# pierremtb/PINNs-TF2.0

Hardware: AMD Instinct MI355X
Metric: collocation-points/sec (higher is better)
Workload: dtype f64

## Files before the change

### pinns-tf2.0_amd/csrc/engine.hip

```cpp
#include <hip/hip_runtime.h>
#include <rccl/rccl.h>

#include <cmath>
#include <cstdarg>
#include <cstddef>
#include <cstdio>
#include <cstring>
#include <string>
#include <chrono>
#include <type_traits>
#include <vector>

#include "../../include/pinn_hip.h"
#include "devbuf.h"
#include "optim_host.h"
#include "kernels_fused20.h"
#include "kernels_fused20m.h"
#include "fused20d_api.h"
#include "fused20m_api.h"
#include "kernels_wide.h"
#include "kernels_generic.h"
#include "kernels_optim.h"
#include "kernels_disc.h"
#include "kernels_sampling.h"
// ... 87 lines not shown

struct pinn_ctx {
  int device = 0, dtype = PINN_F32, pde = PINN_PDE_BURGERS;
  KernelPath path = KP_GENERIC;
  hipStream_t stream = nullptr;
  bool own_stream = true;
  NetDesc nd{};
  int layers[MAX_DENSE + 1]{};
  int n_layers = 0;
  double lb[2]{}, ub[2]{}, nu = 0.0;
  double adr[6]{};
  int adr_mask = 0;

  PointSets sets;
  int64_t nf_total = 0, nu_total = 0, nb_total = 0;
  bool sets_dirty = true;
  SetDesc sd{};

  DevBuf<void> xs, ts, tgt;
  DevBuf<double> theta, gl, adam_m, adam_v;
  DevBuf<void> theta_r;
  DevBuf<float> img;
  DevBuf<int> row_index;
  int n_cu = 256, n_wg = 0;
  int f64_split = -1;
  DevBuf<void> S, O, ZA, ZB, part;
  int chunk = 0, n_rows = 0, R = 0;
  DevBuf<void> xe, te, Oe;
  DevBuf<double> f_out;
  std::vector<double> ev_X, ev_ref;
  int ev_n_pad = 0;
  DevBuf<double> pred, d_ref, err_partial, err_res;
  PinnedBuf<double> h_err;
  DevBuf<unsigned long long> d_nonfinite;
  unsigned long long n_evals = 0;

  struct {
    double lr = 1e-3, b1 = 0.9, b2 = 0.999, eps = 1e-7;
    int64_t t = 0;
    bool ready = false, want_terms = false;
    DevBuf<double> loss_hist;
    size_t hist_stride = 0;
  } adam;

  struct Pending {
    int kind = 0;
    int n = 0;
    int base = 0, issued_upto = 0;
    bool want_terms = false;
    hipEvent_t ev = nullptr;
    PinnedBuf<double> h_loss;
    PinnedBuf<int> h_iter;
    PinnedBuf<LbfgsState> h_state;
  };
  static constexpr int N_SNAP = 4;
  DevBuf<double> snap;
  unsigned snap_valid = 0;
  struct : Tickets { Pending pend[N_PENDING]; } tk;

  struct {
    int issued_at_read = 0;
    DevBuf<LbfgsState> state;
    int flip = 0;
    DevBuf<double> x, d, gold, S, Y, ro, al, q, log_loss;
    DevBuf<int> log_iter;
    int max_iter = 0, ncorr = 0, logged_read = 0;
    double lr = 1.0, tol_fun = 0, tol_x = 0, max_eval = 0;
    int iters_issued = 0;
    bool post_pending = false;
    bool ready = false;
    int mode = 1, mode_active = 0, M1 = 0;
    DevBuf<double> SY, YY, dots, cs, cy;
    DevBuf<LbcExtra> ex;
  } lbfgs;
  double t16_cost_full = T16_COST_FULL, t16_cost_strip = T16_COST_STRIP;
  long long t16_handover_ticks = 50000000ll;
  bool t16_prepass_pinned = false;
  bool t16_prepass = false;
  DevBuf<unsigned int> t16_bsync;
  unsigned int t16_bcount = 0;
  DevBuf<double> t16_gscr;

  enum ColFrom { COL_HANDED, COL_LHS, COL_RAD };
  struct ColOrigin { ColFrom from = COL_HANDED; int64_t n_design = 0, first = 0, count = 0; } col;
  struct { uint64_t seed = 0; } lhs;
  struct {
    bool filled = false;
    DevBuf<double> cx, ct;
    DevBuf<void> px, pt, O;
    DevBuf<double> f;
    DevBuf<unsigned long long> w, bsum;
    DevBuf<RadTotals> tot;
  } rad;

  struct {
    bool on = false;
    double lr = 0.0;
    LamStore arr;
  } sa;
  struct {
    bool on = false;
    double rate[3] = {0.0, 0.0, 0.0};
    LamStore arr;
  } pw;

  struct {
    std::vector<double> X, alpha, beta, g;
    int64_t n_total = 0;
    DevBuf<void> ab;
    int first = 0, n = 0;
    DevBuf<double> out;
  } robin;

  struct {
    std::vector<double> s;
    bool on = false, stale = false;
  } src;

  struct {
    std::vector<double> K;
    bool on = false, stale = false;
    DevBuf<void> dev;
// ... 782 lines not shown
  HIPCHK(hipMemsetAsync(c->part, 0, need_part, c->stream));
  c->dd = dd;
  c->n_rows = G;
  c->sets_dirty = false;
  return 0;
}

template <typename real, int NT>
static int disc_set_lds() {
  static unsigned long long done = 0;
  if (!first_call_on_device(done)) return 0;
  HIPCHK(hipFuncSetAttribute((const void*)k_disc_fwd<real, NT>, hipFuncAttributeMaxDynamicSharedMemorySize,
                             (int)disc_fwd_lds<NT>(sizeof(real))));
  HIPCHK(hipFuncSetAttribute((const void*)k_disc_bwd_out<real, NT>, hipFuncAttributeMaxDynamicSharedMemorySize,
                             (int)disc_out_lds<NT>(sizeof(real))));
  HIPCHK(hipFuncSetAttribute((const void*)k_disc_bwd_hidden<real, NT>, hipFuncAttributeMaxDynamicSharedMemorySize,
                             (int)disc_hid_lds<NT>(sizeof(real))));
  return 0;
}

template <typename real, int NT>
static int disc_eval(pinn_ctx* c, hipEvent_t* ev4, const AdamFuse* af) {
  const DiscDesc dd = c->dd;
  const InMap<real> m(c->lb, c->ub);
  const real c1 = real(1), c2 = (real)c->nu;
  if (int rc = disc_set_lds<real, NT>()) return rc;
  const dim3 grid(dd.n_groups, dd.n_chunks), block(256);
  const real* th = c->theta_r.as<real>();
  if (ev4) HIPCHK(hipEventRecord(ev4[0], c->stream));
  hipLaunchKernelGGL((k_disc_fwd<real, NT>), grid, block, disc_fwd_lds<NT>(sizeof(real)), c->stream, c->nd, dd, th,
                     c->xs.as<real>(), m.lbx, m.sx, c1, c2, c->d_Ast.as<real>(), c->d_A3.as<real>(), c->d_U3.as<real>(),
                     c->d_Nn.as<real>(), 1);
  hipLaunchKernelGGL((k_disc_irk<real>), grid, block, 0, c->stream, dd, c->nd.n_out, c->d_ginfo,
                     c->d_MT[0].as<real>(), c->d_MT[1].as<real>(), c->d_Nn.as<real>(),
                     c->d_U3.as<real>(), c->tgt.as<real>(), c->d_R.as<real>(), c->d_lossp.as<real>(), 0);
  if (ev4) HIPCHK(hipEventRecord(ev4[1], c->stream));
  hipLaunchKernelGGL((k_disc_bwd_out<real, NT>), grid, block, disc_out_lds<NT>(sizeof(real)), c->stream, c->nd, dd,
                     th, c->d_ginfo, c->d_M[0].as<real>(), c->d_M[1].as<real>(), c->d_R.as<real>(),
                     c->d_U3.as<real>(), c->d_A3.as<real>(), c1, c2, c->part.as<real>(), c->R, c->d_dAp.as<real>(),
                     c->d_lamp.as<real>());
  hipLaunchKernelGGL((k_disc_bwd_hidden<real, NT>), dim3(dd.n_groups), block, disc_hid_lds<NT>(sizeof(real)),
                     c->stream, c->nd, dd, th, c->d_ginfo, c->xs.as<real>(), m.lbx, m.sx, c->d_Ast.as<real>(),
                     c->d_dAp.as<real>(), c->d_lossp.as<real>(), c->d_lamp.as<real>(), c->part.as<real>(), c->R);
  if (ev4) HIPCHK(hipEventRecord(ev4[2], c->stream));
  HIPCHK(hipGetLastError());
  return launch_reduce<real>(c, dd.n_groups, af);
}

static int disc_eval_any(pinn_ctx* c, hipEvent_t* ev4, const AdamFuse* af) {
  if (c->dtype == PINN_F64) return disc_eval<double, 4>(c, ev4, af);
  return c->dd.wp == 64 ? disc_eval<float, 4>(c, ev4, af) : disc_eval<float, 8>(c, ev4, af);
}

static int eval_loss_grad(pinn_ctx* c, const AdamFuse* af = nullptr) {
  int rc = src_fresh(c, "evaluation");
  if (rc) return rc;
  rc = is_disc(c) ? disc_ensure(c) : ensure_sets(c);
  if (rc) return rc;
  c->n_evals += 1;
  hipEvent_t* ev4 = nullptr;
  if (c->timing && c->ev_used < c->ev_cap_evals && (c->ev_seen++ % c->ev_every) == 0)
    ev4 = &c->ev[(size_t)4 * c->ev_used];
  if (is_disc(c)) rc = disc_eval_any(c, ev4, af);
  else
    rc = by_kind(c, pde_kind(c, AT_TRAINING), [&](auto r, auto kind) {
      return launch_sweeps<decltype(r), decltype(kind)::value>(c, ev4, af);
    });
  if (rc) return rc;
  if (c->comm && !c->xg.on)
    NCCLCHK(ncclAllReduce(c->gl, c->gl, (size_t)c->R, ncclDouble, ncclSum, c->comm, c->stream));
  if (ev4) { HIPCHK(hipEventRecord(ev4[3], c->stream)); c->ev_used++; }
  return 0;
}

template <typename real, int NT>
static int disc_predict_impl(pinn_ctx* c, int mode, int set, const double* x, int64_t n, double* out) {
  const int NO = c->nd.n_out;
  const int G = (int)((n + 15) / 16);
  DiscDesc dd{};
  disc_layout(c, dd, G, mode == 1 && c->dset[set].has_M ? c->dset[set].q : 0);
  std::vector<double> hx(dd.n_pad, c->lb[0]);
  for (int64_t i = 0; i < n; ++i) hx[i] = x[i];
  std::vector<int> gi(G, disc_ginfo(set, 16));
  DevBuf<void> xe, U3, Nn, Rb;
  DevBuf<int> ge;
  const size_t rs = sizeof(real);
  HIPCHK(xe.reserve_bytes(dd.n_pad * rs));
  HIPCHK(ge.reserve(G));
  if (disc_alloc_scratch(c, dd, nullptr, nullptr, U3, Nn, Rb)) return PINN_EHIP;
  if (upload_real(c, xe, hx.data(), dd.n_pad)) return PINN_EHIP;
  if (hipMemcpy(ge, gi.data(), G * sizeof(int), hipMemcpyHostToDevice) != hipSuccess) return PINN_EHIP;
  const InMap<real> m(c->lb, c->ub);
  const size_t lds_f = disc_fwd_lds<NT>(rs);
  if (int rc = disc_set_lds<real, NT>()) return rc;
  const dim3 grid(dd.n_groups, dd.n_chunks), block(256);
  hipLaunchKernelGGL((k_disc_fwd<real, NT>), grid, block, lds_f, c->stream, c->nd, dd, c->theta_r.as<real>(),
                     xe.as<real>(), m.lbx, m.sx, real(1), (real)c->nu, (real*)nullptr, (real*)nullptr, U3.as<real>(),
                     Nn.as<real>(), 0);
  if (mode == 1)
    hipLaunchKernelGGL((k_disc_irk<real>), grid, block, 0, c->stream, dd, NO, ge.get(), c->d_MT[0].as<real>(),
                       c->d_MT[1].as<real>(), Nn.as<real>(), U3.as<real>(), (const real*)nullptr, Rb.as<real>(),
                       (real*)nullptr, 1);
  std::vector<real> ho((size_t)dd.n_pad * dd.ldo);
  if (hipMemcpyAsync(ho.data(), mode == 1 ? Rb.get() : U3.get(), ho.size() * rs, hipMemcpyDeviceToHost, c->stream) != hipSuccess ||
      hipStreamSynchronize(c->stream) != hipSuccess)
    return fail(PINN_EHIP, "discrete-time predict failed: %s", hipGetErrorString(hipGetLastError()));
  for (int64_t i = 0; i < n; ++i)
    for (int j = 0; j < NO; ++j) out[(size_t)i * NO + j] = (double)ho[(size_t)i * dd.ldo + j];
  return 0;
}

// ... 900 lines not shown
  if (int rc = xg_check(c)) return rc;
  if (losses) {
    if (p.want_terms) memcpy(losses, p.h_loss, (size_t)3 * p.n * 8);
    else for (int s = 0; s < p.n; ++s) losses[s] = p.h_loss[3 * s] + p.h_loss[3 * s + 1] + p.h_loss[3 * s + 2];
  }
  return 0;
}

int pinn_adam_run(pinn_ctx* c, int n_steps, double* losses) {
  REQUIRE(c && n_steps >= 0, "bad arguments");
  if (n_steps == 0) return 0;
  if (!losses) return adam_issue(c, n_steps, false, nullptr);
  REQUIRE(c->tk.outstanding() == 0, "pinn_adam_run: %d chunk(s) are in flight; collect them first", c->tk.outstanding());
  int ticket = 0;
  if (int rc = adam_issue(c, n_steps, true, &ticket)) return rc;
  return pinn_adam_collect(c, ticket, losses);
}

int pinn_adam_enqueue(pinn_ctx* c, int n_steps, int* ticket) {
  REQUIRE(c && ticket && n_steps >= 1, "bad arguments");
  return adam_issue(c, n_steps, true, ticket);
}

int pinn_adam_enqueue_terms(pinn_ctx* c, int n_steps, int* ticket) {
  REQUIRE(c && ticket && n_steps >= 1, "bad arguments");
  c->adam.want_terms = true;
  const int rc = adam_issue(c, n_steps, true, ticket);
  c->adam.want_terms = false;
  return rc;
}

int pinn_adam_run_terms(pinn_ctx* c, int n_steps, double* terms3) {
  REQUIRE(c && terms3, "null");
  c->adam.want_terms = true;
  const int rc = pinn_adam_run(c, n_steps, terms3);
  c->adam.want_terms = false;
  return rc;
}

static int lbfgs_begin_setup(pinn_ctx* c, int max_iter, double lr, int n_corr, double tol_fun, double tol_x,
                             double max_eval, bool* eval) {
  *eval = false;
  REQUIRE(c && max_iter >= 0 && n_corr >= 1 && lr > 0, "bad L-BFGS arguments");
  if (int rc0 = src_fresh(c, "pinn_lbfgs_begin")) return rc0;
  HIPCHK(hipSetDevice(c->device));
  const size_t n = c->nd.n_theta;
  auto& lb = c->lbfgs;
  lb.max_iter = max_iter; lb.lr = lr; lb.ncorr = n_corr; lb.tol_fun = tol_fun; lb.tol_x = tol_x;
  lb.max_eval = max_eval > 0 ? max_eval : 1.25 * max_iter;
  if (c->tk.outstanding() > 0) {
    HIPCHK(hipStreamSynchronize(c->stream));
    c->tk.drop_all();
  }
  lb.iters_issued = 0; lb.logged_read = 0; lb.issued_at_read = 0; lb.post_pending = false; lb.ready = false;
  if (max_iter == 0) { lb.ready = true; return 0; }
  const int M1 = lb.M1 = n_corr + 1;
  lb.mode_active = (lb.mode == 1 && M1 <= LBC_MAXSLOTS) ? 1 : 0;
  if (lb.mode_active && lbc_coef_apply_lds_bytes(M1) > 64 * 1024) {
    const int lds = (int)lbc_coef_apply_lds_bytes(M1);
    HIPCHK(hipFuncSetAttribute((const void*)k_lbc_coef_apply<float>, hipFuncAttributeMaxDynamicSharedMemorySize, lds));
    HIPCHK(hipFuncSetAttribute((const void*)k_lbc_coef_apply<double>, hipFuncAttributeMaxDynamicSharedMemorySize, lds));
  }
  const size_t m1 = M1, ring = m1 * ring_ld((int)n), gram = 2 * m1 * m1, dots = 2 * (5 * m1 + LBC_NSCAL);
  const struct { DevBuf<double>* buf; size_t count; bool zero; } bufs[] = {
      {&lb.x, n, false},    {&lb.d, n, false},    {&lb.gold, n, false},  {&lb.q, n, false},     {&lb.al, m1, false},
      {&lb.S, ring, true},  {&lb.Y, ring, true},  {&lb.cs, m1, true},    {&lb.cy, m1, true},    {&lb.SY, gram, true},
      {&lb.YY, gram, true}, {&lb.ro, 2 * m1, true}, {&lb.dots, dots, true}};
  static_assert(sizeof(LbcExtra) % 8 == 0, "LbcExtra is cleared as doubles");
  ZeroList zl{};
  auto add = [&](void* p, size_t doubles) { zl.p[zl.count] = (double*)p; zl.n[zl.count] = doubles; zl.count++; };
  for (const auto& b : bufs) {
    HIPCHK(b.buf->reserve(b.count));
    if (b.zero) add(b.buf->get(), b.count);
  }
  HIPCHK(lb.state.reserve(2));
  HIPCHK(lb.ex.reserve(1));
  add(lb.ex, sizeof(LbcExtra) / 8);
  static_assert(sizeof(LbfgsState) % 8 == 0 && offsetof(LbfgsState, Hdiag) % 8 == 0, "LbfgsState is initialised as doubles");
  zl.state = (double*)lb.state.get(); zl.state_doubles = (int)(sizeof(LbfgsState) / 8);
  zl.hdiag_index = (int)(offsetof(LbfgsState, Hdiag) / 8);
  hipLaunchKernelGGL(k_zero_list, dim3(256), dim3(256), 0, c->stream, zl);
  HIPCHK(hipGetLastError());
  lb.flip = 0;
  HIPCHK(lb.log_loss.reserve((size_t)max_iter + 1));
  HIPCHK(lb.log_iter.reserve((size_t)max_iter + 1));
  HIPCHK(hipMemcpyAsync(lb.x, c->theta, n * 8, hipMemcpyDeviceToDevice, c->stream));
  *eval = true;
  return 0;
}

static void lbfgs_post(pinn_ctx* c, int initial) {
  const auto& lb = c->lbfgs;
  const int n = c->nd.n_theta;
  hipLaunchKernelGGL(k_lbfgs_post, dim3(1), dim3(LB_THREADS), 0, c->stream, n, n, lb.max_iter, lb.max_eval, lb.tol_fun,
                     lb.tol_x, lb.state + lb.flip, c->gl, lb.d, lb.log_iter, lb.log_loss, initial);
}

static int lbfgs_begin_post(pinn_ctx* c) {
  lbfgs_post(c, 1);
  HIPCHK(hipGetLastError());
  if (c->xg.on) {
    HIPCHK(hipStreamSynchronize(c->stream));
    if (int rc2 = xg_check(c)) return rc2;
  }
  c->lbfgs.ready = true;
  return 0;
}

int pinn_lbfgs_begin(pinn_ctx* c, int max_iter, double lr, int n_corr, double tol_fun,
                     double tol_x, double max_eval) {
  bool eval = false;
  if (int rc = lbfgs_begin_setup(c, max_iter, lr, n_corr, tol_fun, tol_x, max_eval, &eval)) return rc;
  if (!eval) return 0;
  if (int rc = eval_loss_grad(c)) return rc;
  return lbfgs_begin_post(c);
}

struct LbfgsMember { pinn_ctx* c; pinn_ctx::Pending* p; int window, ticket; };

static int lbfgs_open(LbfgsMember& m, int n_iters) {
  pinn_ctx* c = m.c;
  REQUIRE(c && n_iters >= 0, "bad arguments");
  if (int rc0 = src_fresh(c, "pinn_lbfgs_run / pinn_lbfgs_enqueue")) return rc0;
  const auto& lb = c->lbfgs;
  REQUIRE(lb.ready, "pinn_lbfgs_begin has not been called");
  HIPCHK(hipSetDevice(c->device));
  pinn_ctx::Pending* p = nullptr;
  const int log_room = (int)(lb.log_iter.capacity_bytes() / sizeof(int));
  const int window = lbfgs_window(lb.iters_issued, lb.issued_at_read, n_iters, log_room, lb.logged_read, lb.max_iter);
  if (int rc = pend_reserve(c, 2, (size_t)window + 1, (size_t)window + 1, true, &p)) return rc;
  if (lb.max_iter == 0) { p->n = -1; return ticket_issue(c, p, &m.ticket); }
  m.p = p; m.window = window;
  return 0;
}

static bool lbfgs_iter(pinn_ctx* c) {
  auto& lb = c->lbfgs;
  const int n = c->nd.n_theta;
  lb.iters_issued += 1;
  if (lb.mode_active) {
    const int M1 = lb.M1;
    const size_t lsh = lbc_coef_apply_lds_bytes(M1), mm = (size_t)M1 * M1;
    LbfgsState *st_in = lb.state + lb.flip, *st_out = lb.state + (lb.flip ^ 1);
    const int n_part = n <= 2 * 2 * LBD_THREADS ? 2 : 1;
    if (n_part == 2)
      hipLaunchKernelGGL(k_lbc_dots<2>, dim3(M1, 2), dim3(LBD_THREADS), 0, c->stream, n, M1, st_in, c->gl, lb.gold, lb.d,
                         lb.S, lb.Y, lb.dots);
    else
      hipLaunchKernelGGL(k_lbc_dots<1>, dim3(M1), dim3(LBD_THREADS), 0, c->stream, n, M1, st_in, c->gl, lb.gold, lb.d,
                         lb.S, lb.Y, lb.dots);
    const double* pd = lb.dots;
    const dim3 agrid((n + 63) / 64);
    by_real(c, [&](auto r) {
      using real = decltype(r);
      hipLaunchKernelGGL((k_lbc_coef_apply<real>), agrid, dim3(LBC_THREADS), lsh, c->stream, n, M1, lb.ncorr, lb.max_iter,
                         lb.lr, lb.tol_x, lb.tol_fun, lb.max_eval, lb.post_pending ? 1 : 0, n, st_in, st_out, c->gl, pd,
                         n_part, lb.SY + lb.flip * mm, lb.YY + lb.flip * mm, lb.ro + lb.flip * M1,
                         lb.SY + (lb.flip ^ 1) * mm, lb.YY + (lb.flip ^ 1) * mm, lb.ro + (lb.flip ^ 1) * M1, lb.log_iter,
                         lb.log_loss, lb.S, lb.Y, lb.d, lb.gold, lb.x, c->theta, c->theta_r.as<real>(), c->nd, c->img);
    });
    lb.post_pending = false;
    lb.flip ^= 1;
  } else
    by_real(c, [&](auto r) {
      using real = decltype(r);
      hipLaunchKernelGGL((k_lbfgs_step<real>), dim3(1), dim3(LB_THREADS), 0, c->stream, n, lb.max_iter, lb.ncorr,
                         lb.lr, lb.tol_x, lb.state + lb.flip, c->gl, lb.x, c->theta, c->theta_r.as<real>(),
                         lb.d, lb.gold, lb.S, lb.Y, lb.ro, lb.al, lb.q, c->nd, c->img);
    });
  return lb.iters_issued != lb.max_iter;
}

static int lbfgs_close(LbfgsMember& m) {
  pinn_ctx* c = m.c;
  auto& lb = c->lbfgs;
  pinn_ctx::Pending* p = m.p;
  if (lb.post_pending) { lbfgs_post(c, 0); lb.post_pending = false; }
  HIPCHK(hipGetLastError());
  p->n = m.window; p->base = lb.logged_read; p->issued_upto = lb.iters_issued;
  HIPCHK(hipMemcpyAsync(p->h_state, lb.state + lb.flip, sizeof(LbfgsState), hipMemcpyDeviceToHost, c->stream));
  if (m.window > 0) {
    HIPCHK(hipMemcpyAsync(p->h_iter, lb.log_iter + p->base, (size_t)m.window * 4, hipMemcpyDeviceToHost, c->stream));
    HIPCHK(hipMemcpyAsync(p->h_loss, lb.log_loss + p->base, (size_t)m.window * 8, hipMemcpyDeviceToHost, c->stream));
  }
  return ticket_issue(c, p, &m.ticket);
}

extern "C++" {
template <typename Eval>
static int lbfgs_chunk(LbfgsMember* m, char* act, int K, int n_iters, Eval&& eval) {
  for (int k = 0; k < K; ++k)
    if (int rc = lbfgs_open(m[k], n_iters)) return rc;
  for (int s = 0; s < n_iters; ++s) {
    bool any = false;
    for (int k = 0; k < K; ++k) {
      pinn_ctx* c = m[k].c;
      act[k] = m[k].p && c->lbfgs.iters_issued < c->lbfgs.max_iter && lbfgs_iter(c);
      any = any || act[k];
    }
    if (!any) break;
    if (int rc = eval(act)) return rc;
    for (int k = 0; k < K; ++k) {
      if (!act[k]) continue;
      if (m[k].c->lbfgs.mode_active) m[k].c->lbfgs.post_pending = true;
      else lbfgs_post(m[k].c, 0);
    }
  }
  for (int k = 0; k < K; ++k)
    if (m[k].p) { if (int rc = lbfgs_close(m[k])) return rc; }
  return 0;
}
}

static int lbfgs_issue(pinn_ctx* c, int n_iters, int* ticket) {
  const Range rg("pinn_lbfgs_run");
  LbfgsMember m{c, nullptr, 0, 0};
  char act = 0;
  if (int rc = lbfgs_chunk(&m, &act, 1, n_iters, [c](const char*) { return eval_loss_grad(c); })) return rc;
  *ticket = m.ticket;
  return 0;
}

int pinn_lbfgs_collect(pinn_ctx* c, int ticket, int cap, int* iters, double* losses, int* n_logged, int* done) {
  REQUIRE(cap >= 0, "bad arguments");
  pinn_ctx::Pending* pp = nullptr;
  if (int rc = ticket_oldest(c, ticket, 2, &pp)) return rc;
  const pinn_ctx::Pending& p = *pp;
  auto& lb = c->lbfgs;
  if (n_logged) *n_logged = 0;
  if (p.n < 0) { if (done) *done = 1; return 0; }
  if (int rc2 = xg_check(c)) return rc2;
  const LbfgsState hs = *p.h_state;
  const LbfgsHandout h = lbfgs_handout(hs.n_logged, lb.logged_read, p.base, p.n);
  REQUIRE(!(iters && losses) || h.fresh <= cap, "pinn_lbfgs_collect: %d log entries are due, the arrays hold %d", h.fresh, cap);
  if (h.fresh > 0 && iters && losses) {
    if (!h.inside)
      return fail(PINN_ESTATE, "pinn_lbfgs_collect: log entries from %d on lie outside the chunk's window of %d", h.off, p.n);
    memcpy(iters, p.h_iter + h.off, (size_t)h.fresh * 4);
    memcpy(losses, p.h_loss + h.off, (size_t)h.fresh * 8);
  }
  lb.logged_read = hs.n_logged;
  lb.issued_at_read = p.issued_upto;
  if (n_logged) *n_logged = (iters && losses) ? h.fresh : 0;
  if (done) *done = hs.done;
  return 0;
}

int pinn_lbfgs_run(pinn_ctx* c, int n_iters, int* iters, double* losses, int* n_logged, int* done) {
  REQUIRE(c && n_iters >= 0, "bad arguments");
  REQUIRE(c->tk.outstanding() == 0, "pinn_lbfgs_run: %d chunk(s) are in flight; collect them first", c->tk.outstanding());
  int ticket = 0;
  if (int rc = lbfgs_issue(c, n_iters, &ticket)) return rc;
  return pinn_lbfgs_collect(c, ticket, n_iters, iters, losses, n_logged, done);
}

int pinn_lbfgs_enqueue(pinn_ctx* c, int n_iters, int* ticket) {
  REQUIRE(c && ticket && n_iters >= 1, "bad arguments");
  return lbfgs_issue(c, n_iters, ticket);
}

int pinn_lbfgs_set_mode(pinn_ctx* c, int mode) {
  REQUIRE(c && (mode == 0 || mode == 1), "mode must be 0 (reference operation order) or 1 (compact)");
  c->lbfgs.mode = mode;
  return 0;
}

int pinn_lbfgs_get_x(pinn_ctx* c, double* x, int64_t n) {
  REQUIRE(c && x && n == c->nd.n_theta, "bad arguments");
  REQUIRE(c->lbfgs.x, "no L-BFGS run yet");
  HIPCHK(hipSetDevice(c->device));
  HIPCHK(hipMemcpyAsync(x, c->lbfgs.x, (size_t)n * 8, hipMemcpyDeviceToHost, c->stream));
  HIPCHK(hipStreamSynchronize(c->stream));
  return 0;
}

int pinn_predict(pinn_ctx* c, const double* X, int64_t n, double* out) {
  REQUIRE(c && X && out && n >= 0, "bad arguments");
  HIPCHK(hipSetDevice(c->device));
  if (n == 0) return 0;
  if (is_disc(c))
    return disc_predict_any(c, 0, 0, X, n, out);
  const Range rg("pinn_predict");
  int n_pad = 0;
  if (int rc = eval_points(c, X, n, &n_pad)) return rc;
  if (int rc = predict_values(c, n, n_pad)) return rc;
  HIPCHK(hipMemcpyAsync(out, c->pred, (size_t)n * c->nd.n_out * 8, hipMemcpyDeviceToHost, c->stream));
  HIPCHK(hipStreamSynchronize(c->stream));
  return 0;
}

int pinn_error_l2(pinn_ctx* c, const double* X, const double* ref, int64_t n, int kind, double* err) {
  REQUIRE(c && X && ref && err && n >= 1, "bad arguments");
// ... 930 lines not shown
}

int pinn_ens_adam_init(pinn_ens* e, double lr, double beta1, double beta2, double eps, const double* lr_k) {
  REQUIRE(e, "null");
  for (int k = 0; k < e->K; ++k)
    if (int rc = pinn_adam_init(e->mem[k], lr_k ? lr_k[k] : lr, beta1, beta2, eps)) return rc;
  return 0;
}

int pinn_ens_adam_run(pinn_ens* e, int n_steps, double* losses) {
  REQUIRE(e && n_steps >= 0, "bad arguments");
  for (pinn_ctx* c : e->mem) REQUIRE(c->adam.ready, "pinn_ens_adam_init has not been called");
  pinn_ctx* b = e->base;
  HIPCHK(hipSetDevice(b->device));
  if (n_steps == 0) return 0;
  const size_t K = e->K;
  HIPCHK(e->loss_hist.reserve((size_t)n_steps * K * 3));
  std::vector<char> all(K, 1);
  std::vector<double> alpha(K);
  for (int s = 0; s < n_steps; ++s) {
    for (size_t k = 0; k < K; ++k)
      alpha[k] = adam_step_factors(e->mem[k]).alpha(e->mem[k]->adam.lr);
    if (int rc = ens_eval(e, (const bool*)all.data(), alpha.data(), e->loss_hist + (size_t)s * K * 3)) return rc;
  }
  std::vector<double> h((size_t)n_steps * K * 3);
  HIPCHK(hipMemcpyAsync(h.data(), e->loss_hist, h.size() * 8, hipMemcpyDeviceToHost, b->stream));
  HIPCHK(hipStreamSynchronize(b->stream));
  if (losses)
    for (size_t i = 0; i < (size_t)n_steps * K; ++i) losses[i] = h[3 * i] + h[3 * i + 1] + h[3 * i + 2];
  return 0;
}

int pinn_ens_lbfgs_begin(pinn_ens* e, int n_corr, double tol_fun, double tol_x, double max_eval, double lr,
                         const double* lr_k, int max_iter, const int* max_iter_k) {
  REQUIRE(e, "null");
  REQUIRE(n_corr >= 1, "bad L-BFGS arguments");
  for (int k = 0; k < e->K; ++k) {
    REQUIRE((lr_k ? lr_k[k] : lr) > 0 && (max_iter_k ? max_iter_k[k] : max_iter) >= 0,
            "bad L-BFGS arguments for member %d", k);
  }
  HIPCHK(hipSetDevice(e->base->device));
  std::vector<char> ev((size_t)e->K, 0);
  bool any = false;
  for (int k = 0; k < e->K; ++k) {
    bool eval = false;
    if (int rc = lbfgs_begin_setup(e->mem[k], max_iter_k ? max_iter_k[k] : max_iter, lr_k ? lr_k[k] : lr, n_corr,
                                   tol_fun, tol_x, max_eval, &eval)) return rc;
    ev[k] = eval;
    any = any || eval;
  }
  if (!any) return 0;
  if (int rc = ens_eval(e, (const bool*)ev.data(), nullptr, nullptr)) return rc;
  for (int k = 0; k < e->K; ++k)
    if (ev[k]) { if (int rc = lbfgs_begin_post(e->mem[k])) return rc; }
  return 0;
}

int pinn_ens_lbfgs_run(pinn_ens* e, int n_iters, int* iters, double* losses, int* n_logged, int* done) {
  REQUIRE(e && n_iters >= 0, "bad arguments");
  for (pinn_ctx* c : e->mem) {
    REQUIRE(c->lbfgs.ready, "pinn_ens_lbfgs_begin has not been called");
    REQUIRE(c->tk.outstanding() == 0, "chunks in flight");
  }
  HIPCHK(hipSetDevice(e->base->device));
  const Range rg("pinn_ens_lbfgs_run");
  const int K = e->K;
  std::vector<LbfgsMember> m(K);
  for (int k = 0; k < K; ++k) m[k].c = e->mem[k];
  std::vector<char> act(K, 0);
  if (int rc = lbfgs_chunk(m.data(), act.data(), K, n_iters,
                           [e](const char* a) { return ens_eval(e, (const bool*)a, nullptr, nullptr); })) return rc;
  const int ld = n_iters + 1;
  for (int k = 0; k < K; ++k) {
    int nl = 0, dn = 0;
    if (int rc = pinn_lbfgs_collect(m[k].c, m[k].ticket, n_iters, iters ? iters + (size_t)k * ld : nullptr,
                               losses ? losses + (size_t)k * ld : nullptr, &nl, &dn)) return rc;
    if (n_logged) n_logged[k] = nl;
    if (done) done[k] = dn;
  }
  return 0;
}

int pinn_ens_predict(pinn_ens* e, const double* X, int64_t n, double* out) {
  REQUIRE(e && X && out && n >= 0, "bad arguments");
  for (int k = 0; k < e->K; ++k)
    if (int rc = pinn_predict(e->mem[k], X, n, out + (size_t)k * n)) return rc;
  return 0;
}

int pinn_ens_error_l2(pinn_ens* e, const double* X, const double* ref, int64_t n, double* err) {
  REQUIRE(e && X && ref && err && n > 0, "bad arguments");
  for (int k = 0; k < e->K; ++k)
    if (int rc = pinn_error_l2(e->mem[k], X, ref, n, 0, err + k)) return rc;
  return 0;
}

int pinn_ens_get_status(pinn_ens* e, int64_t* n_evals, int64_t* first_nonfinite_eval) {
  REQUIRE(e, "null");
  for (int k = 0; k < e->K; ++k) {
    int64_t a = 0, b = 0;
    if (int rc = pinn_get_status(e->mem[k], &a, &b)) return rc;
    if (n_evals) n_evals[k] = a;
    if (first_nonfinite_eval) first_nonfinite_eval[k] = b;
  }
  return 0;
}

// ... 2 lines not shown
```

### pinns-tf2.0_amd/csrc/kernels_optim.h

```cpp
#pragma once
#include "kernels_wide.h"

namespace pinn {

#ifndef PINN_REDUCE_ONE_ROUND
#define PINN_REDUCE_ONE_ROUND 1
#endif
constexpr int RED_COLS = 64;
constexpr int RED_SLICES = 16;
constexpr int RED_THREADS = RED_COLS * RED_SLICES;

template <typename real>
__device__ __forceinline__ double reduce_column(const real* __restrict__ part, int n_rows, int R,
                                                int c, int q, double (*sh)[RED_COLS]) {
  const int cl = threadIdx.x & 63;
  double a0 = 0, a1 = 0, a2 = 0, a3 = 0, a4 = 0, a5 = 0, a6 = 0, a7 = 0;
  if (c < R) {
#if PINN_REDUCE_ONE_ROUND
    const unsigned lane_off = (unsigned)c * (unsigned)sizeof(real);
    for (int r0 = __builtin_amdgcn_readfirstlane(q); r0 < n_rows; r0 += 16 * RED_SLICES) {
      real v[16];
#pragma unroll
      for (int i = 0; i < 16; ++i)
        v[i] = (r0 + i * RED_SLICES < n_rows)
// ... 384 lines not shown
    const double xi = x[i] + t * d[i];
    x[i] = xi;
    if (will_eval) { theta[i] = xi; theta_r[i] = (real)xi; pack_store_any(nd, img, i, (float)xi); }
  }
  if (tid == 0) {
    st->n_iter = n_iter; st->hist_len = hist_len; st->hist_head = head; st->Hdiag = Hdiag;
    st->t = t; st->f_old = st->f;
    if (!will_eval) st->done = 1;
  }
}

__global__ __launch_bounds__(LB_THREADS) void k_lbfgs_post(
    int n, int n_theta, int max_iter, double max_eval, double tol_fun, double tol_x,
    LbfgsState* __restrict__ st, const double* __restrict__ gl, const double* __restrict__ d,
    int* __restrict__ log_iters, double* __restrict__ log_losses, int initial) {
  __shared__ double sh[LB_THREADS / 64];
  if (st->done) return;
  const int tid = threadIdx.x;
  const double f = gl[n_theta] + gl[n_theta + 1] + gl[n_theta + 2];
  double ga_p = 0, sa_p = 0;
  const double t = st->t;
  for (int i = tid; i < n; i += LB_THREADS) {
    ga_p += fabs(gl[i]);
    if (!initial) sa_p += fabs(d[i] * t);
  }
  const double gabs = block_sum(ga_p, sh);
  const double sabs = block_sum(sa_p, sh);
  if (tid != 0) return;
  if (initial) {
    st->f = f; st->func_eval = 1;
    if (gabs <= tol_fun) st->done = 7;
    return;
  }
  const double f_old = st->f_old;
  st->f = f;
  st->func_eval += 1;
  const int n_iter = st->n_iter;
  if (n_iter == max_iter) { st->done = 1; return; }
  if ((double)st->func_eval >= max_eval) { st->done = 3; return; }
  if (gabs <= tol_fun) { st->done = 4; return; }
  if (sabs <= tol_x) { st->done = 5; return; }
  if (fabs(f - f_old) < tol_x) { st->done = 6; return; }
  const int k = st->n_logged;
  log_iters[k] = n_iter;
  log_losses[k] = f;
  st->n_logged = k + 1;
  if (n_iter == max_iter - 1) st->final_loss = f;
}

struct LbcExtra {
  int apply, will_eval, pad0, pad1;
  double cg, gtd;
};

struct ZeroList {
  double* p[10];
  unsigned long long n[10];
  int count;
  double* state;
  int state_doubles, hdiag_index;
};
__global__ __launch_bounds__(256) void k_zero_list(ZeroList zl) {
  if (zl.state && blockIdx.x == 0 && threadIdx.x == 0)
    for (int i = 0; i < zl.state_doubles; ++i) zl.state[i] = i == zl.hdiag_index ? 1.0 : 0.0;
  for (int a = 0; a < zl.count; ++a) {
    double* __restrict__ p = zl.p[a];
    const unsigned long long n = zl.n[a];
    for (unsigned long long i = (unsigned long long)blockIdx.x * 256 + threadIdx.x; i < n;
         i += (unsigned long long)gridDim.x * 256)
      p[i] = 0.0;
  }
}

constexpr int LBC_THREADS = 1024;
constexpr int LBC_ROWS = 4;
constexpr int LBD_THREADS = 1024;
constexpr int LBC_NSCAL = 5;

template <int NV>
__device__ __forceinline__ void block_sums(double (&v)[NV], double (*sh)[8]) {
  const int w = threadIdx.x >> 6;
#pragma unroll
  for (int i = 0; i < NV; ++i) {
    const double t = wave_sum(v[i]);
    if ((threadIdx.x & 63) == 0) sh[w][i] = t;
  }
  __syncthreads();
#pragma unroll
  for (int i = 0; i < NV; ++i) {
    double t = 0;
#pragma unroll
    for (int k = 0; k < LBD_THREADS / 64; ++k) t += sh[k][i];
    v[i] = t;
  }
}

template <int HALVES>
__global__ __launch_bounds__(LBD_THREADS) void k_lbc_dots(
    int n, int M1, const LbfgsState* __restrict__ st, const double* __restrict__ g,
    const double* __restrict__ g_old, const double* __restrict__ d, double* __restrict__ Sh,
    double* __restrict__ Yh, double* __restrict__ dots_all) {
  __shared__ double sh[LBD_THREADS / 64][8];
  double* __restrict__ dots = dots_all + (HALVES == 2 ? blockIdx.y * (5 * M1 + LBC_NSCAL) : 0);
  const int u0 = HALVES == 2 ? (int)blockIdx.y : 0;
  constexpr int NS = HALVES == 2 ? 1 : 2;
  typedef double d2 __attribute__((ext_vector_type(2)));
  const int a = blockIdx.x, tid = threadIdx.x;
  const int done0 = st->done, head = st->hist_head, len = st->hist_len, n_it = st->n_iter;
  const double t = st->t;
  d2 gv[NS], gov[NS], dv[NS], sav[NS], yav[NS];
#pragma unroll
  for (int u = 0; u < NS; ++u) {
    const int i = 2 * tid + (u0 + u) * 2 * LBD_THREADS;
    const d2 z = {0.0, 0.0};
    gv[u] = gov[u] = dv[u] = sav[u] = yav[u] = z;
    if (i + 1 < n) {
      gv[u] = *reinterpret_cast<const d2*>(g + i); gov[u] = *reinterpret_cast<const d2*>(g_old + i);
// ... 87 lines not shown
  extern __shared__ double lsh[];
  const int tid = threadIdx.x, lane = tid & 63, wave = uni(tid >> 6);
  const bool writer = blockIdx.x == 0;
  const int LD = M1 | 1;
  double* const sU = lsh;
  double* const sL = sU + M1 * LD;
  double* const sY = sL + M1 * LD;
  double* const sT = sY + M1 * LD;
  double* const sC = sT + 6 * 64;
  double* const sP = sC + 192;
  double* const sZ = sP + 16 * 64;
  CSTAMP(0);
  const bool in_row = lane < M1;
  const LbfgsState s0 = *st_in;
  int head = uni(s0.hist_head), len = uni(s0.hist_len);
  double Hdiag = s0.Hdiag, f_cur = s0.f;
  const int ndp = 5 * M1 + LBC_NSCAL;
  double ys = pd[5 * M1 + 0], yy = pd[5 * M1 + 1], gg = pd[5 * M1 + 2], gabs = pd[5 * M1 + 3], sabs = pd[5 * M1 + 4];
  double qv = (wave < 5 && in_row) ? pd[wave * M1 + lane] : 0.0;
  if (n_part == 2) {
    const double* __restrict__ p2 = pd + ndp;
    ys += p2[5 * M1 + 0]; yy += p2[5 * M1 + 1]; gg += p2[5 * M1 + 2]; gabs += p2[5 * M1 + 3]; sabs += p2[5 * M1 + 4];
    qv += (wave < 5 && in_row) ? p2[wave * M1 + lane] : 0.0;
  }
  const double ro_l0 = in_row ? ro_in[lane] : 0.0;
  const double f_new = gl[n_theta] + gl[n_theta + 1] + gl[n_theta + 2];
  double ra[LBC_ROWS], rb[LBC_ROWS];
#pragma unroll
  for (int u = 0; u < LBC_ROWS; ++u) {
    const int r = wave + 16 * u;
    const bool ok = r < M1 && in_row;
    ra[u] = ok ? SY_in[r * M1 + lane] : 0.0;
    rb[u] = ok ? YY_in[r * M1 + lane] : 0.0;
  }
  const int i = blockIdx.x * 64 + lane;
  const bool iok = i < n;
  const double gi = (iok && wave == 0) ? gl[i] : 0.0, xi0 = (iok && wave == 0) ? x[i] : 0.0;
  double yv[4] = {0.0, 0.0, 0.0, 0.0}, sv[4] = {0.0, 0.0, 0.0, 0.0};
  auto fetch_history = [&]() {
#pragma unroll
    for (int u = 0; u < 4; ++u) {
      const int sl = wave + 16 * u;
      const bool ok = iok && sl < M1;
      yv[u] = ok ? Yh[(size_t)sl * ring_ld(n) + i] : 0.0;
      sv[u] = ok ? Sh[(size_t)sl * ring_ld(n) + i] : 0.0;
    }
  };
  if (wave == 0) fetch_history();
  const int done0 = uni(s0.done);
  if (done0) { if (writer && tid == 0) *st_out = s0; return; }
  CSTAMP(1);
  LbfgsState s1 = s0;
  int dn = 0;
  if (do_post) {
    f_cur = f_new;
    if (s0.n_iter == max_iter) dn = 1;
    else if ((double)(s0.func_eval + 1) >= max_eval) dn = 3;
    else if (gabs <= tol_fun) dn = 4;
    else if (sabs <= tol_x) dn = 5;
    else if (fabs(f_cur - s0.f_old) < tol_x) dn = 6;
    s1.f = f_cur; s1.func_eval = s0.func_eval + 1;
    if (dn) s1.done = dn;
    else {
      if (writer && tid == 0) { log_iters[s0.n_logged] = s0.n_iter; log_losses[s0.n_logged] = f_cur; }
      s1.n_logged = s0.n_logged + 1;
      if (s0.n_iter == max_iter - 1) s1.final_loss = f_cur;
    }
  }
  if (dn) { if (writer && tid == 0) *st_out = s1; return; }

  const int n_iter = s0.n_iter + 1;
  const bool first = (n_iter == 1);
  int c = head + len; if (c >= M1) c -= M1;
  const bool accept = !first && ys > 1e-10;
  if (accept) {
    Hdiag = ys / yy;
    if (len == m) { head += 1; if (head >= M1) head -= M1; } else len += 1;
  }
  const double ro_l = (accept && lane == c) ? 1.0 / ys : ro_l0;
  if (wave < 5) sT[wave * 64 + lane] = !in_row ? 0.0 : qv;
  if (wave == 5) {
    sT[5 * 64 + lane] = ro_l;
    if (writer && in_row) ro_out[lane] = ro_l;
    sZ[lane] = 0.0;
  }
  if (wave == 1 && LD > M1 && in_row) {
    sU[lane * LD + M1] = 0.0; sL[lane * LD + M1] = 0.0; sY[lane * LD + M1] = 0.0;
  }
  lds_barrier();
  CSTAMP(2);
  {
    int pb = lane - head; if (pb < 0) pb += M1;
    const bool vb = in_row && pb < len;
    const bool lc = accept && lane == c;
    const double d_sya = sT[1 * 64 + lane], d_yya = sT[2 * 64 + lane];
    double ro_r[LBC_ROWS], say_r[LBC_ROWS], yya_r[LBC_ROWS];
#pragma unroll
    for (int u = 0; u < LBC_ROWS; ++u) {
      const int r = wave + 16 * u, rr = r < M1 ? r : 0;
      ro_r[u] = sT[5 * 64 + rr]; say_r[u] = sT[0 * 64 + rr]; yya_r[u] = sT[2 * 64 + rr];
    }
#pragma unroll
    for (int u = 0; u < LBC_ROWS; ++u) {
      const int r = wave + 16 * u;
      if (r < M1) {
        const bool rc = accept && r == c;
        const double sy = rc ? (lc ? ys : d_sya) : (lc ? say_r[u] : ra[u]);
// ... 124 lines not shown
```

### pinns-tf2.0_amd/csrc/optim_host.h

```cpp
#pragma once
#include <cmath>
#include <cstddef>

namespace pinn {

constexpr int N_PENDING = 4;

struct Tickets {
  unsigned long long issued = 0, collected = 0;
  int outstanding() const { return (int)(issued - collected); }
  bool room() const { return outstanding() < N_PENDING; }
  int next_slot() const { return (int)(issued % N_PENDING); }
  int next_number() const { return (int)(issued & 0x7fffffff); }
  int oldest_slot() const { return (int)(collected % N_PENDING); }
  bool is_oldest(int ticket) const { return outstanding() > 0 && ticket == (int)(collected & 0x7fffffff); }
  void drop_all() { collected = issued; }
};

struct AdamFactors {
  double s, d;
  AdamFactors(double b1, double b2, double t) : s(std::sqrt(1.0 - std::pow(b2, t))), d(1.0 - std::pow(b1, t)) {}
  double alpha(double lr) const { return lr * s / d; }
  double bc_pw() const { return s / d; }
};

inline size_t ring_steps(int n_steps) { return n_steps < 16 ? 16 : (size_t)n_steps; }
inline size_t ring_doubles(size_t steps) { return steps * N_PENDING * 3; }
inline bool ring_must_grow(size_t steps, size_t capacity_bytes) { return ring_doubles(steps) * 8 > capacity_bytes; }
inline size_t ring_region(const Tickets& tk, size_t stride) { return (size_t)tk.next_slot() * stride * 3; }

inline int lbfgs_window(int iters_issued, int issued_at_read, int n_iters, int log_room, int logged_read, int max_iter) {
  int window = (iters_issued - issued_at_read) + n_iters + 1;
  if (window > log_room - logged_read) window = log_room - logged_read;
  if (window < 0 || max_iter == 0) window = 0;
  return window;
}

struct LbfgsHandout { int off, fresh; bool inside; };
inline LbfgsHandout lbfgs_handout(int n_logged, int logged_read, int base, int window) {
  const int fresh = n_logged > logged_read ? n_logged - logged_read : 0;
  const int off = logged_read - base;
  return {off, fresh, off >= 0 && off + fresh <= window};
}

}
```

Baseline: 236.6 million.

## Pack L-BFGS readback into one buffer and fold initial post into first step

```diff
diff --git a/pinns-tf2.0_amd/csrc/engine.hip b/pinns-tf2.0_amd/csrc/engine.hip
--- a/pinns-tf2.0_amd/csrc/engine.hip
+++ b/pinns-tf2.0_amd/csrc/engine.hip
@@ -163,6 +163,10 @@
     PinnedBuf<double> h_loss;
     PinnedBuf<int> h_iter;
     PinnedBuf<LbfgsState> h_state;
+    PinnedBuf<char> h_span;
+    const LbfgsState* r_state = nullptr;
+    const int* r_iter = nullptr;
+    const double* r_loss = nullptr;
   };
   static constexpr int N_SNAP = 4;
   DevBuf<double> snap;
@@ -171,14 +175,17 @@
 
   struct {
     int issued_at_read = 0;
+    DevBuf<char> readback;
     DevBuf<LbfgsState> state;
     int flip = 0;
-    DevBuf<double> x, d, gold, S, Y, ro, al, q, log_loss;
+    DevBuf<double> x, d, gold, S, Y, ro, al, q;
+    DevBuf<double> log_loss;
     DevBuf<int> log_iter;
+    int log_room = 0;
     int max_iter = 0, ncorr = 0, logged_read = 0;
     double lr = 1.0, tol_fun = 0, tol_x = 0, max_eval = 0;
     int iters_issued = 0;
-    bool post_pending = false;
+    int post_pending = LBC_POST_NONE;
     bool ready = false;
     int mode = 1, mode_active = 0, M1 = 0;
     DevBuf<double> SY, YY, dots, cs, cy;
@@ -1067,11 +1074,13 @@
   return c->dd.wp == 64 ? disc_eval<float, 4>(c, ev4, af) : disc_eval<float, 8>(c, ev4, af);
 }
 
+static void lbfgs_settle(pinn_ctx* c);
 static int eval_loss_grad(pinn_ctx* c, const AdamFuse* af = nullptr) {
   int rc = src_fresh(c, "evaluation");
   if (rc) return rc;
   rc = is_disc(c) ? disc_ensure(c) : ensure_sets(c);
   if (rc) return rc;
+  if (c->lbfgs.post_pending == LBC_POST_INITIAL) lbfgs_settle(c);
   c->n_evals += 1;
   hipEvent_t* ev4 = nullptr;
   if (c->timing && c->ev_used < c->ev_cap_evals && (c->ev_seen++ % c->ev_every) == 0)
@@ -2078,12 +2087,13 @@
     HIPCHK(hipStreamSynchronize(c->stream));
     c->tk.drop_all();
   }
-  lb.iters_issued = 0; lb.logged_read = 0; lb.issued_at_read = 0; lb.post_pending = false; lb.ready = false;
+  lb.iters_issued = 0; lb.logged_read = 0; lb.issued_at_read = 0; lb.post_pending = LBC_POST_NONE; lb.ready = false;
   if (max_iter == 0) { lb.ready = true; return 0; }
   const int M1 = lb.M1 = n_corr + 1;
   lb.mode_active = (lb.mode == 1 && M1 <= LBC_MAXSLOTS) ? 1 : 0;
-  if (lb.mode_active && lbc_coef_apply_lds_bytes(M1) > 64 * 1024) {
-    const int lds = (int)lbc_coef_apply_lds_bytes(M1);
+  static unsigned long long attr = 0;
+  if (lb.mode_active && first_call_on_device(attr)) {
+    const int lds = (int)lbc_coef_apply_lds_bytes(LBC_MAXSLOTS);
     HIPCHK(hipFuncSetAttribute((const void*)k_lbc_coef_apply<float>, hipFuncAttributeMaxDynamicSharedMemorySize, lds));
     HIPCHK(hipFuncSetAttribute((const void*)k_lbc_coef_apply<double>, hipFuncAttributeMaxDynamicSharedMemorySize, lds));
   }
@@ -2099,18 +2109,24 @@
     HIPCHK(b.buf->reserve(b.count));
     if (b.zero) add(b.buf->get(), b.count);
   }
-  HIPCHK(lb.state.reserve(2));
+  HIPCHK(lb.readback.reserve_bytes(LbfgsReadback::bytes(sizeof(LbfgsState), (size_t)max_iter + 1)));
+  {
+    const LbfgsReadback rb{sizeof(LbfgsState), LbfgsReadback::room_of(sizeof(LbfgsState), lb.readback.capacity_bytes())};
+    char* base = lb.readback.get();
+    lb.state.borrow((LbfgsState*)(base + rb.state_at(0)));
+    lb.log_loss.borrow((double*)(base + rb.loss_at(0)));
+    lb.log_iter.borrow((int*)(base + rb.iter_at(0)));
+    lb.log_room = (int)rb.room;
+  }
   HIPCHK(lb.ex.reserve(1));
   add(lb.ex, sizeof(LbcExtra) / 8);
   static_assert(sizeof(LbfgsState) % 8 == 0 && offsetof(LbfgsState, Hdiag) % 8 == 0, "LbfgsState is initialised as doubles");
   zl.state = (double*)lb.state.get(); zl.state_doubles = (int)(sizeof(LbfgsState) / 8);
   zl.hdiag_index = (int)(offsetof(LbfgsState, Hdiag) / 8);
+  zl.copy_src = c->theta; zl.copy_dst = lb.x; zl.copy_n = n;
   hipLaunchKernelGGL(k_zero_list, dim3(256), dim3(256), 0, c->stream, zl);
   HIPCHK(hipGetLastError());
   lb.flip = 0;
-  HIPCHK(lb.log_loss.reserve((size_t)max_iter + 1));
-  HIPCHK(lb.log_iter.reserve((size_t)max_iter + 1));
-  HIPCHK(hipMemcpyAsync(lb.x, c->theta, n * 8, hipMemcpyDeviceToDevice, c->stream));
   *eval = true;
   return 0;
 }
@@ -2122,7 +2138,15 @@
                      lb.tol_x, lb.state + lb.flip, c->gl, lb.d, lb.log_iter, lb.log_loss, initial);
 }
 
-static int lbfgs_begin_post(pinn_ctx* c) {
+static void lbfgs_settle(pinn_ctx* c) {
+  auto& lb = c->lbfgs;
+  if (lb.post_pending == LBC_POST_NONE) return;
+  lbfgs_post(c, lb.post_pending == LBC_POST_INITIAL ? 1 : 0);
+  lb.post_pending = LBC_POST_NONE;
+}
+
+static int lbfgs_begin_post(pinn_ctx* c, bool fold) {
+  if (fold && c->lbfgs.mode_active && !c->comm && !c->xg.on) { c->lbfgs.post_pending = LBC_POST_INITIAL; c->lbfgs.ready = true; return 0; }
   lbfgs_post(c, 1);
   HIPCHK(hipGetLastError());
   if (c->xg.on) {
@@ -2139,7 +2163,7 @@
   if (int rc = lbfgs_begin_setup(c, max_iter, lr, n_corr, tol_fun, tol_x, max_eval, &eval)) return rc;
   if (!eval) return 0;
   if (int rc = eval_loss_grad(c)) return rc;
-  return lbfgs_begin_post(c);
+  return lbfgs_begin_post(c, true);
 }
 
 struct LbfgsMember { pinn_ctx* c; pinn_ctx::Pending* p; int window, ticket; };
@@ -2152,9 +2176,9 @@
   REQUIRE(lb.ready, "pinn_lbfgs_begin has not been called");
   HIPCHK(hipSetDevice(c->device));
   pinn_ctx::Pending* p = nullptr;
-  const int log_room = (int)(lb.log_iter.capacity_bytes() / sizeof(int));
-  const int window = lbfgs_window(lb.iters_issued, lb.issued_at_read, n_iters, log_room, lb.logged_read, lb.max_iter);
+  const int window = lbfgs_window(lb.iters_issued, lb.issued_at_read, n_iters, lb.log_room, lb.logged_read, lb.max_iter);
   if (int rc = pend_reserve(c, 2, (size_t)window + 1, (size_t)window + 1, true, &p)) return rc;
+  HIPCHK(p->h_span.reserve_bytes(LBFGS_ONE_COPY_BYTES));
   if (lb.max_iter == 0) { p->n = -1; return ticket_issue(c, p, &m.ticket); }
   m.p = p; m.window = window;
   return 0;
@@ -2180,12 +2204,12 @@
     by_real(c, [&](auto r) {
       using real = decltype(r);
       hipLaunchKernelGGL((k_lbc_coef_apply<real>), agrid, dim3(LBC_THREADS), lsh, c->stream, n, M1, lb.ncorr, lb.max_iter,
-                         lb.lr, lb.tol_x, lb.tol_fun, lb.max_eval, lb.post_pending ? 1 : 0, n, st_in, st_out, c->gl, pd,
+                         lb.lr, lb.tol_x, lb.tol_fun, lb.max_eval, lb.post_pending, n, st_in, st_out, c->gl, pd,
                          n_part, lb.SY + lb.flip * mm, lb.YY + lb.flip * mm, lb.ro + lb.flip * M1,
                          lb.SY + (lb.flip ^ 1) * mm, lb.YY + (lb.flip ^ 1) * mm, lb.ro + (lb.flip ^ 1) * M1, lb.log_iter,
                          lb.log_loss, lb.S, lb.Y, lb.d, lb.gold, lb.x, c->theta, c->theta_r.as<real>(), c->nd, c->img);
     });
-    lb.post_pending = false;
+    lb.post_pending = LBC_POST_NONE;
     lb.flip ^= 1;
   } else
     by_real(c, [&](auto r) {
@@ -2201,14 +2225,25 @@
   pinn_ctx* c = m.c;
   auto& lb = c->lbfgs;
   pinn_ctx::Pending* p = m.p;
-  if (lb.post_pending) { lbfgs_post(c, 0); lb.post_pending = false; }
+  lbfgs_settle(c);
   HIPCHK(hipGetLastError());
   p->n = m.window; p->base = lb.logged_read; p->issued_upto = lb.iters_issued;
+  const LbfgsReadback rb{sizeof(LbfgsState), (size_t)lb.log_room};
+  const LbfgsSpan sp = lbfgs_span(rb, lb.flip, p->base, m.window);
+  if (sp.bytes <= LBFGS_ONE_COPY_BYTES) {
+    char* h = p->h_span;
+    HIPCHK(hipMemcpyAsync(h, lb.readback + sp.begin, sp.bytes, hipMemcpyDeviceToHost, c->stream));
+    p->r_state = (const LbfgsState*)h;
+    p->r_loss = (const double*)(h + (rb.loss_at(p->base) - sp.begin));
+    p->r_iter = (const int*)(h + (rb.iter_at(p->base) - sp.begin));
+    return ticket_issue(c, p, &m.ticket);
+  }
   HIPCHK(hipMemcpyAsync(p->h_state, lb.state + lb.flip, sizeof(LbfgsState), hipMemcpyDeviceToHost, c->stream));
   if (m.window > 0) {
     HIPCHK(hipMemcpyAsync(p->h_iter, lb.log_iter + p->base, (size_t)m.window * 4, hipMemcpyDeviceToHost, c->stream));
     HIPCHK(hipMemcpyAsync(p->h_loss, lb.log_loss + p->base, (size_t)m.window * 8, hipMemcpyDeviceToHost, c->stream));
   }
+  p->r_state = p->h_state; p->r_iter = p->h_iter; p->r_loss = p->h_loss;
   return ticket_issue(c, p, &m.ticket);
 }
 
@@ -2228,7 +2263,7 @@
     if (int rc = eval(act)) return rc;
     for (int k = 0; k < K; ++k) {
       if (!act[k]) continue;
-      if (m[k].c->lbfgs.mode_active) m[k].c->lbfgs.post_pending = true;
+      if (m[k].c->lbfgs.mode_active) m[k].c->lbfgs.post_pending = LBC_POST_STEP;
       else lbfgs_post(m[k].c, 0);
     }
   }
@@ -2256,14 +2291,14 @@
   if (n_logged) *n_logged = 0;
   if (p.n < 0) { if (done) *done = 1; return 0; }
   if (int rc2 = xg_check(c)) return rc2;
-  const LbfgsState hs = *p.h_state;
+  const LbfgsState hs = *p.r_state;
   const LbfgsHandout h = lbfgs_handout(hs.n_logged, lb.logged_read, p.base, p.n);
   REQUIRE(!(iters && losses) || h.fresh <= cap, "pinn_lbfgs_collect: %d log entries are due, the arrays hold %d", h.fresh, cap);
   if (h.fresh > 0 && iters && losses) {
     if (!h.inside)
       return fail(PINN_ESTATE, "pinn_lbfgs_collect: log entries from %d on lie outside the chunk's window of %d", h.off, p.n);
-    memcpy(iters, p.h_iter + h.off, (size_t)h.fresh * 4);
-    memcpy(losses, p.h_loss + h.off, (size_t)h.fresh * 8);
+    memcpy(iters, p.r_iter + h.off, (size_t)h.fresh * 4);
+    memcpy(losses, p.r_loss + h.off, (size_t)h.fresh * 8);
   }
   lb.logged_read = hs.n_logged;
   lb.issued_at_read = p.issued_upto;
@@ -3300,7 +3335,7 @@
   if (!any) return 0;
   if (int rc = ens_eval(e, (const bool*)ev.data(), nullptr, nullptr)) return rc;
   for (int k = 0; k < e->K; ++k)
-    if (ev[k]) { if (int rc = lbfgs_begin_post(e->mem[k])) return rc; }
+    if (ev[k]) { if (int rc = lbfgs_begin_post(e->mem[k], false)) return rc; }
   return 0;
 }
 
diff --git a/pinns-tf2.0_amd/csrc/kernels_optim.h b/pinns-tf2.0_amd/csrc/kernels_optim.h
--- a/pinns-tf2.0_amd/csrc/kernels_optim.h
+++ b/pinns-tf2.0_amd/csrc/kernels_optim.h
@@ -460,6 +460,7 @@
   int apply, will_eval, pad0, pad1;
   double cg, gtd;
 };
+constexpr int LBC_POST_NONE = 0, LBC_POST_STEP = 1, LBC_POST_INITIAL = 2;
 
 struct ZeroList {
   double* p[10];
@@ -467,10 +468,20 @@
   int count;
   double* state;
   int state_doubles, hdiag_index;
+  const double* copy_src;
+  double* copy_dst;
+  unsigned long long copy_n;
 };
 __global__ __launch_bounds__(256) void k_zero_list(ZeroList zl) {
   if (zl.state && blockIdx.x == 0 && threadIdx.x == 0)
     for (int i = 0; i < zl.state_doubles; ++i) zl.state[i] = i == zl.hdiag_index ? 1.0 : 0.0;
+  {
+    const double* __restrict__ s = zl.copy_src;
+    double* __restrict__ q = zl.copy_dst;
+    for (unsigned long long i = (unsigned long long)blockIdx.x * 256 + threadIdx.x; i < zl.copy_n;
+         i += (unsigned long long)gridDim.x * 256)
+      q[i] = s[i];
+  }
   for (int a = 0; a < zl.count; ++a) {
     double* __restrict__ p = zl.p[a];
     const unsigned long long n = zl.n[a];
@@ -664,7 +675,11 @@
   CSTAMP(1);
   LbfgsState s1 = s0;
   int dn = 0;
-  if (do_post) {
+  if (do_post == LBC_POST_INITIAL) {
+    f_cur = f_new;
+    s1.f = f_cur; s1.func_eval = 1;
+    if (gabs <= tol_fun) s1.done = dn = 7;
+  } else if (do_post) {
     f_cur = f_new;
     if (s0.n_iter == max_iter) dn = 1;
     else if ((double)(s0.func_eval + 1) >= max_eval) dn = 3;
diff --git a/pinns-tf2.0_amd/csrc/optim_host.h b/pinns-tf2.0_amd/csrc/optim_host.h
--- a/pinns-tf2.0_amd/csrc/optim_host.h
+++ b/pinns-tf2.0_amd/csrc/optim_host.h
@@ -43,4 +43,23 @@
   return {off, fresh, off >= 0 && off + fresh <= window};
 }
 
+struct LbfgsReadback {
+  size_t state_bytes;
+  size_t room;
+  static size_t bytes(size_t state_bytes, size_t room) { return 2 * state_bytes + room * 12; }
+  static size_t room_of(size_t state_bytes, size_t capacity_bytes) {
+    return capacity_bytes > 2 * state_bytes ? (capacity_bytes - 2 * state_bytes) / 12 : 0;
+  }
+  size_t state_at(int flip) const { return (size_t)flip * state_bytes; }
+  size_t loss_at(size_t entry) const { return 2 * state_bytes + entry * 8; }
+  size_t iter_at(size_t entry) const { return 2 * state_bytes + room * 8 + entry * 4; }
+};
+constexpr size_t LBFGS_ONE_COPY_BYTES = 16 * 1024;
+struct LbfgsSpan { size_t begin, bytes; };
+inline LbfgsSpan lbfgs_span(const LbfgsReadback& rb, int flip, int base, int window) {
+  const size_t begin = rb.state_at(flip);
+  const size_t end = window > 0 ? rb.iter_at((size_t)base + (size_t)window) : begin + rb.state_bytes;
+  return {begin, end - begin};
 }
+
+}
```

Measured after the change: 236.3 million. About the same (-0.1%).
